# PengfeiRen96/DIR

Measured on AMD Instinct MI355X. Metric: images/sec at 256x256 bs=64, 3 stage outputs (DIR.forward eval), higher is better.
Workload: dtype f16

## Files before the change

### dir_amd/csrc/bneck.hip

```cpp
#include "conv_common.h"

#ifndef DIR_BNECK_RES16
#define DIR_BNECK_RES16 1
#endif

namespace dir {
namespace {

using convk::bf16_t;
using convk::f16s_t;
using convk::Half;
using convk::f32x16;
typedef __attribute__((ext_vector_type(4))) float f32x4;

constexpr int TH = 8, TW = 16, NPX = TH * TW;
constexpr int PH = TH + 2, PWD = TW + 2, NPP = PH * PWD;
constexpr int PPITCH = 144;
constexpr int W2PITCH = 1168;
constexpr int TPITCH = 528;
constexpr int NTHR = 512;
constexpr int NPRE = (NPP * 8 + NTHR - 1) / NTHR;

struct ChainArgs {
    const bf16_t* y1; const bf16_t* res; bf16_t* out; bf16_t* y1n;
    const bf16_t* w2; const float* sc2; const float* sh2;
    const bf16_t* w3; const float* sc3; const float* sh3;
    const bf16_t* w1n; const float* sc1n; const float* sh1n;
    const bf16_t* x2; const bf16_t* wd;
    int B, H, W, tiles_x, tiles_y, ntiles;
    int decim;
};

template <typename H> __device__ __forceinline__ void unpack4(uint2 v, float (&f)[4]) {
    convk::unpack2<H>(v.x, f[0], f[1]);
    convk::unpack2<H>(v.y, f[2], f[3]);
}

template <bool HAS_RES, int N2, bool HAS_DUAL, typename H = bf16_t>
__global__ __launch_bounds__(NTHR, 1) void bneck_chain_kernel(ChainArgs a) {
    convk::half_kernel_init<H>();
    constexpr bool HAS_NEXT = N2 > 0;
    __shared__ __attribute__((aligned(16))) char s_w2[64 * W2PITCH];
    __shared__ __attribute__((aligned(16))) char s_patch[NPP * PPITCH];
    __shared__ __attribute__((aligned(16))) char s_y2[NPX * PPITCH];
    __shared__ __attribute__((aligned(16))) char s_t[64 * TPITCH];
    __shared__ __attribute__((aligned(16))) float s_ss[896];
    const int tid = threadIdx.x, lane = tid & 63, wave = __builtin_amdgcn_readfirstlane(tid >> 6);
    const int l32 = lane & 31, h = lane >> 5;
    const int l16 = lane & 15, g = lane >> 4;

    for (int c = tid; c < 64 * 72; c += NTHR) {
        const int row = c / 72, col = c - row * 72;
        *reinterpret_cast<uint4*>(s_w2 + row * W2PITCH + col * 16) = *reinterpret_cast<const uint4*>(a.w2 + row * 576 + col * 8);
    }
    if (tid < 64) { s_ss[tid] = a.sc2[tid]; s_ss[64 + tid] = a.sh2[tid]; }
    if (tid < 256) { s_ss[128 + tid] = a.sc3[tid]; s_ss[384 + tid] = a.sh3[tid]; }
    if (HAS_NEXT && tid < N2) { s_ss[640 + tid] = a.sc1n[tid]; s_ss[768 + tid] = a.sh1n[tid]; }
    convk::u32x4 w3f[4];
#pragma unroll
    for (int s = 0; s < 4; ++s) w3f[s] = *reinterpret_cast<const convk::u32x4*>(a.w3 + (32 * wave + l32) * 64 + 16 * s + 8 * h);
    convk::u32x4 wdf[HAS_DUAL ? 4 : 1];
    if constexpr (HAS_DUAL) {
#pragma unroll
        for (int s = 0; s < 4; ++s) wdf[s] = *reinterpret_cast<const convk::u32x4*>(a.wd + (32 * wave + l32) * 64 + 16 * s + 8 * h);
    }
    constexpr int NPT = N2 == 128 ? 4 : 2;
    const int ct = N2 == 128 ? wave : (wave >> 1), pt0 = N2 == 128 ? 0 : 2 * (wave & 1);
    convk::u32x4 w1f[HAS_NEXT ? 8 : 1];
    if constexpr (HAS_NEXT) {
#pragma unroll
        for (int s = 0; s < 8; ++s) w1f[s] = *reinterpret_cast<const convk::u32x4*>(a.w1n + (16 * ct + l16) * 256 + 32 * s + 8 * g);
    }

    const int nblk = gridDim.x;
    int t0, tstep, tend;
    if ((nblk & 7) == 0 && a.ntiles % 8 == 0) {
        const int per = a.ntiles >> 3;
        t0 = (blockIdx.x & 7) * per + (blockIdx.x >> 3); tstep = nblk >> 3; tend = ((blockIdx.x & 7) + 1) * per;
    } else { t0 = blockIdx.x; tstep = nblk; tend = a.ntiles; }

    uint4 pre[NPRE];
    unsigned okmask = 0;
    auto origin = [&](int t, int& b, int& y0, int& x0) {
        const int tx = t % a.tiles_x, r = t / a.tiles_x;
        b = r / a.tiles_y; y0 = (r - b * a.tiles_y) * TH; x0 = tx * TW;
    };
    auto fetch = [&](int t) {
        int b, y0, x0;
        origin(t, b, y0, x0);
        okmask = 0;
#pragma unroll
        for (int i = 0; i < NPRE; ++i) {
            const int e = tid + NTHR * i, pp = e >> 3, cc = e & 7;
            const int pr = pp / PWD, pc = pp - pr * PWD;
            const int iy = y0 - 1 + pr, ix = x0 - 1 + pc;
            if (e < NPP * 8 && iy >= 0 && iy < a.H && ix >= 0 && ix < a.W) okmask |= 1u << i;
            const int iyc = min(max(iy, 0), a.H - 1), ixc = min(max(ix, 0), a.W - 1);
            pre[i] = *reinterpret_cast<const uint4*>(a.y1 + (((long long)b * a.H + iyc) * a.W + ixc) * 64 + cc * 8);
        }
    };
    auto stage = [&]() {
#pragma unroll
        for (int i = 0; i < NPRE; ++i) {
            const int e = tid + NTHR * i, pp = e >> 3, cc = e & 7;
            if (e < NPP * 8)
                *reinterpret_cast<uint4*>(s_patch + pp * PPITCH + cc * 16) = (okmask >> i) & 1u ? pre[i] : make_uint4(0u, 0u, 0u, 0u);
        }
    };

    int t = t0;
    if (t < tend) fetch(t);
#pragma unroll
    for (int s = 0; s < 4; ++s) asm volatile("" ::"v"(w3f[s]));
    if constexpr (HAS_DUAL) {
#pragma unroll
        for (int s = 0; s < 4; ++s) asm volatile("" ::"v"(wdf[s]));
    }
    if constexpr (HAS_NEXT) {
#pragma unroll
        for (int s = 0; s < 8; ++s) asm volatile("" ::"v"(w1f[s]));
    }
    if (t < tend) stage();
    __syncthreads();

    const int mt = wave >> 1, nt = wave & 1;
    const int prow = 2 * mt + (l32 >> 4), pcol = l32 & 15;
    const char* pa_b = s_patch + (prow * PWD + pcol) * PPITCH + 16 * h;
    const char* pa_w = s_w2 + (32 * nt + l32) * W2PITCH + 16 * h;

#if DIR_BNECK_RES16
    uint4 xr[2][2][2];
#else
    uint2 xr[2][2][4];
#endif
    auto out_ptr = [&](int mg, int i, int rb, int ry0, int rx0) {
        const int c = tid + NTHR * i, P = 64 * mg + (c >> 5);
        return a.out + (((long long)rb * a.H + ry0 + (P >> 4)) * a.W + rx0 + (P & 15)) * 256 + (c & 31) * 8;
    };

    auto tile = [&](int t) {
        int b, y0, x0;
        origin(t, b, y0, x0);
        const bool more = t + tstep < tend;
        fetch(more ? t + tstep : t);
        if constexpr (HAS_RES) {
#pragma unroll
            for (int mg = 0; mg < 2; ++mg)
#pragma unroll
                for (int j = 0; j < 2; ++j) {
                    const int P = 64 * mg + 32 * j + l32;
#if DIR_BNECK_RES16
                    const bf16_t* rp = a.res + (((long long)b * a.H + y0 + (P >> 4)) * a.W + x0 + (P & 15)) * 256 + 32 * wave + 8 * h;
#pragma unroll
                    for (int jj = 0; jj < 2; ++jj) xr[mg][j][jj] = *reinterpret_cast<const uint4*>(rp + 16 * jj);
#else
                    const bf16_t* rp = a.res + (((long long)b * a.H + y0 + (P >> 4)) * a.W + x0 + (P & 15)) * 256 + 32 * wave + 4 * h;
#pragma unroll
                    for (int q = 0; q < 4; ++q) xr[mg][j][q] = *reinterpret_cast<const uint2*>(rp + 8 * q);
#endif
                }
        }

        uint4 xq0 = make_uint4(0u, 0u, 0u, 0u), xq1 = xq0;
        if constexpr (HAS_DUAL) {
            const int P0 = tid >> 3, P1 = (tid + NTHR) >> 3;
            xq0 = *reinterpret_cast<const uint4*>(a.x2 + (((long long)b * a.H + y0 + (P0 >> 4)) * a.W + x0 + (P0 & 15)) * 64 + (tid & 7) * 8);
            xq1 = *reinterpret_cast<const uint4*>(a.x2 + (((long long)b * a.H + y0 + (P1 >> 4)) * a.W + x0 + (P1 & 15)) * 64 + (tid & 7) * 8);
        }

        {
            f32x16 acc;
#pragma unroll
            for (int r = 0; r < 16; ++r) acc[r] = 0.f;
            uint4 wv[3], pv[3];
            auto ldfrag = [&](int i, int slot) {
                const int tap = i >> 2, s = i & 3, ky = tap / 3, kx = tap - 3 * ky;
                wv[slot] = *reinterpret_cast<const uint4*>(pa_w + tap * 128 + 32 * s);
                pv[slot] = *reinterpret_cast<const uint4*>(pa_b + (ky * PWD + kx) * PPITCH + 32 * s);
            };
            ldfrag(0, 0);
            ldfrag(1, 1);
#pragma unroll
            for (int i = 0; i < 36; ++i) {
                if (i + 2 < 36) ldfrag(i + 2, (i + 2) % 3);
                __builtin_amdgcn_sched_barrier(0);
                acc = Half<H>::mfma32(wv[i % 3], pv[i % 3], acc);
                __builtin_amdgcn_sched_barrier(0);
            }
#pragma unroll
            for (int q = 0; q < 4; ++q) {
                const int c0 = 32 * nt + 8 * q + 4 * h;
                const float4 sc = *reinterpret_cast<const float4*>(s_ss + c0);
                const float4 sh = *reinterpret_cast<const float4*>(s_ss + 64 + c0);
                uint2 o;
                o.x = Half<H>::pack2_relu(fmaf(acc[4 * q], sc.x, sh.x), fmaf(acc[4 * q + 1], sc.y, sh.y));
                o.y = Half<H>::pack2_relu(fmaf(acc[4 * q + 2], sc.z, sh.z), fmaf(acc[4 * q + 3], sc.w, sh.w));
                *reinterpret_cast<uint2*>(s_y2 + (32 * mt + l32) * PPITCH + c0 * 2) = o;
            }
        }
        __syncthreads();
        if constexpr (HAS_DUAL) {
            *reinterpret_cast<uint4*>(s_patch + (tid >> 3) * PPITCH + (tid & 7) * 16) = xq0;
            *reinterpret_cast<uint4*>(s_patch + ((tid + NTHR) >> 3) * PPITCH + (tid & 7) * 16) = xq1;
            __syncthreads();
        }

#pragma unroll
        for (int mg = 0; mg < 2; ++mg) {
            f32x16 accb[2];
            uint4 pvb[2][4];
#pragma unroll
            for (int j = 0; j < 2; ++j)
#pragma unroll
                for (int s = 0; s < 4; ++s)
                    pvb[j][s] = *reinterpret_cast<const uint4*>(s_y2 + (64 * mg + 32 * j + l32) * PPITCH + 32 * s + 16 * h);
#pragma unroll
            for (int j = 0; j < 2; ++j)
#pragma unroll
                for (int r = 0; r < 16; ++r) accb[j][r] = 0.f;
#pragma unroll
            for (int s = 0; s < 4; ++s)
#pragma unroll
                for (int j = 0; j < 2; ++j) accb[j] = Half<H>::mfma32(w3f[s], pvb[j][s], accb[j]);
            if constexpr (HAS_DUAL) {
#pragma unroll
                for (int j = 0; j < 2; ++j)
#pragma unroll
                    for (int s = 0; s < 4; ++s)
                        pvb[j][s] = *reinterpret_cast<const uint4*>(s_patch + (64 * mg + 32 * j + l32) * PPITCH + 32 * s + 16 * h);
#pragma unroll
                for (int s = 0; s < 4; ++s)
#pragma unroll
                    for (int j = 0; j < 2; ++j) accb[j] = Half<H>::mfma32(wdf[s], pvb[j][s], accb[j]);
            }
#pragma unroll
            for (int j = 0; j < 2; ++j) {
#pragma unroll
                for (int q = 0; q < 4; ++q) {
                    const int c0 = 32 * wave + 8 * q + 4 * h;
                    char* tp = s_t + (32 * j + l32) * TPITCH + c0 * 2;
                    const float4 sc = *reinterpret_cast<const float4*>(s_ss + 128 + c0);
                    const float4 sh = *reinterpret_cast<const float4*>(s_ss + 384 + c0);
                    float v[4] = {fmaf(accb[j][4 * q], sc.x, sh.x), fmaf(accb[j][4 * q + 1], sc.y, sh.y),
                                  fmaf(accb[j][4 * q + 2], sc.z, sh.z), fmaf(accb[j][4 * q + 3], sc.w, sh.w)};
                    if constexpr (HAS_RES) {
                        float rv[4];
#if DIR_BNECK_RES16
                        const uint4 c = xr[mg][j][q >> 1];
                        const auto sx = __builtin_amdgcn_permlane32_swap(c.x, c.z, false, false);
                        const auto sy = __builtin_amdgcn_permlane32_swap(c.y, c.w, false, false);
                        unpack4<H>(make_uint2(sx[q & 1], sy[q & 1]), rv);
#else
                        unpack4<H>(xr[mg][j][q], rv);
#endif
#pragma unroll
                        for (int e = 0; e < 4; ++e) v[e] += rv[e];
                    }
                    uint2 o;
                    o.x = Half<H>::pack2_relu(v[0], v[1]);
                    o.y = Half<H>::pack2_relu(v[2], v[3]);
                    *reinterpret_cast<uint2*>(tp) = o;
                }
            }
            __syncthreads();
            if (!a.decim) {
#pragma unroll
                for (int i = 0; i < 4; ++i) {
                    const int c = tid + NTHR * i;
                    *reinterpret_cast<uint4*>(out_ptr(mg, i, b, y0, x0)) = *reinterpret_cast<const uint4*>(s_t + (c >> 5) * TPITCH + (c & 31) * 16);
                }
            } else {
#pragma unroll
                for (int i = 0; i < 4; ++i) {
                    const int c = tid + NTHR * i, P = 64 * mg + (c >> 5), py = P >> 4, px = P & 15;
                    if (((py | px) & 1) == 0)
                        *reinterpret_cast<uint4*>(a.out + (((long long)b * (a.H >> 1) + ((y0 + py) >> 1)) * (a.W >> 1) + ((x0 + px) >> 1)) * 256 + (c & 31) * 8) =
                            *reinterpret_cast<const uint4*>(s_t + (c >> 5) * TPITCH + (c & 31) * 16);
                }
            }
            if constexpr (HAS_NEXT) {
                f32x4 accc[NPT];
#pragma unroll
                for (int u = 0; u < NPT; ++u) accc[u] = f32x4{0.f, 0.f, 0.f, 0.f};
#pragma unroll
                for (int s = 0; s < 8; ++s)
#pragma unroll
                    for (int u = 0; u < NPT; ++u) {
                        const uint4 pv = *reinterpret_cast<const uint4*>(s_t + (16 * (pt0 + u) + l16) * TPITCH + 64 * s + 16 * g);
                        accc[u] = Half<H>::mfma16(w1f[s], pv, accc[u]);
                    }
                const int c0 = 16 * ct + 4 * g;
                const float4 sc = *reinterpret_cast<const float4*>(s_ss + 640 + c0);
                const float4 sh = *reinterpret_cast<const float4*>(s_ss + 768 + c0);
#pragma unroll
                for (int u = 0; u < NPT; ++u) {
                    const int P = 64 * mg + 16 * (pt0 + u) + l16;
                    uint2 o;
                    o.x = Half<H>::pack2_relu(fmaf(accc[u][0], sc.x, sh.x), fmaf(accc[u][1], sc.y, sh.y));
                    o.y = Half<H>::pack2_relu(fmaf(accc[u][2], sc.z, sh.z), fmaf(accc[u][3], sc.w, sh.w));
                    *reinterpret_cast<uint2*>(a.y1n + (((long long)b * a.H + y0 + (P >> 4)) * a.W + x0 + (P & 15)) * N2 + c0) = o;
                }
            }
            if (mg == 0) __syncthreads();
        }
        stage();
        __syncthreads();
    };
    for (; t < tend; t += tstep) tile(t);
}

}
}

extern "C" int dir_bottleneck_chain_forward(const dir_bneck_chain_params* p, const void* y1, const void* residual, const void* x2, void* out,
                                            void* y1_next, int B, int H, int W, void* stream) {
    using namespace dir;
    DIR_REQUIRE(p && y1 && out && B > 0, "dir_bottleneck_chain_forward: bad args");
    DIR_REQUIRE(p->w2 && p->scale2 && p->shift2 && p->w3 && p->scale3 && p->shift3, "dir_bottleneck_chain_forward: missing conv2 / conv3 parameters");
    DIR_REQUIRE(H > 0 && W > 0 && H % TH == 0 && W % TW == 0, "dir_bottleneck_chain_forward: H must be a multiple of 8 and W of 16");
    const bool next = y1_next != nullptr;
    const bool dual = x2 != nullptr;
    DIR_REQUIRE(!dual || (p->wd && !residual), "dir_bottleneck_chain_forward: a second source needs wd and excludes the identity residual");
    DIR_REQUIRE(!next || (p->w1n && p->scale1n && p->shift1n), "dir_bottleneck_chain_forward: y1_next needs the next conv1 parameters");
    ChainArgs a;
    a.y1 = (const convk::bf16_t*)y1; a.res = (const convk::bf16_t*)residual; a.out = (convk::bf16_t*)out; a.y1n = (convk::bf16_t*)y1_next;
    a.w2 = (const convk::bf16_t*)p->w2; a.sc2 = p->scale2; a.sh2 = p->shift2;
    a.w3 = (const convk::bf16_t*)p->w3; a.sc3 = p->scale3; a.sh3 = p->shift3;
    a.w1n = (const convk::bf16_t*)p->w1n; a.sc1n = p->scale1n; a.sh1n = p->shift1n;
    a.x2 = (const convk::bf16_t*)x2; a.wd = (const convk::bf16_t*)p->wd;
    a.B = B; a.H = H; a.W = W; a.tiles_x = W / TW; a.tiles_y = H / TH; a.decim = p->out_decimate ? 1 : 0;
    const long long nt = (long long)B * a.tiles_x * a.tiles_y;
    DIR_REQUIRE(nt < (1ll << 31) && (long long)B * H * W * 256 < (1ll << 40), "dir_bottleneck_chain_forward: too large");
    a.ntiles = (int)nt;
    static int num_cu = 0;
    if (!num_cu) {
        int dev = 0; hipDeviceProp_t pr;
        num_cu = (hipGetDevice(&dev) == hipSuccess && hipGetDeviceProperties(&pr, dev) == hipSuccess) ? pr.multiProcessorCount : 256;
    }
    const int grid = (int)(nt < num_cu ? nt : num_cu);
    hipStream_t s = (hipStream_t)stream;
    const bool res = residual != nullptr;
    const int n2 = next ? p->n_next : 0;
    DIR_REQUIRE(n2 == 0 || n2 == 64 || n2 == 128, "dir_bottleneck_chain_forward: n_next must be 64 or 128");
    DIR_REQUIRE(p->dtype == 0 || p->dtype == DIR_DT_BF16 || p->dtype == DIR_DT_F16, "dir_bottleneck_chain_forward: dtype must be bf16 (or 0) or f16");
    const bool f16 = p->dtype == DIR_DT_F16;
#define DIR_CHAIN(RES_, N2_, DUAL_) do { if (f16) DIR_LAUNCH((bneck_chain_kernel<RES_, N2_, DUAL_, f16s_t>), dim3(grid), dim3(NTHR), 0, s, a); \
                                         else DIR_LAUNCH((bneck_chain_kernel<RES_, N2_, DUAL_, bf16_t>), dim3(grid), dim3(NTHR), 0, s, a); } while (0)
    if (dual) { if (n2 == 128) DIR_CHAIN(false, 128, true); else if (n2) DIR_CHAIN(false, 64, true); else DIR_CHAIN(false, 0, true); }
    else if (res) { if (n2 == 128) DIR_CHAIN(true, 128, false); else if (n2) DIR_CHAIN(true, 64, false); else DIR_CHAIN(true, 0, false); }
    else { if (n2 == 128) DIR_CHAIN(false, 128, false); else if (n2) DIR_CHAIN(false, 64, false); else DIR_CHAIN(false, 0, false); }
#undef DIR_CHAIN
    return check_launch("dir_bottleneck_chain_forward");
}
```

Measured before the change: 28380.

## Batch bottleneck weight preload, template decimation, and hoist residual lane swaps

Loads the conv2 weights and scale/shift vectors into registers before the first patch fetch, so all global loads go out together before they are written to shared memory. Turns output decimation into a template parameter and rewrites the decimated store so every thread writes one vector without a branch. Computes the residual permlane swaps once per row group instead of once per output quad. Adds an optional, disabled-by-default path that issues the next tile's residual and x2 loads early; this costs more registers and adds template instantiations.

```diff
diff --git a/dir_amd/csrc/bneck.hip b/dir_amd/csrc/bneck.hip
--- a/dir_amd/csrc/bneck.hip
+++ b/dir_amd/csrc/bneck.hip
@@ -1,5 +1,11 @@
 #include "conv_common.h"
 
+#ifndef DIR_BNECK_BATCH
+#define DIR_BNECK_BATCH 1
+#endif
+#ifndef DIR_BNECK_LEAD
+#define DIR_BNECK_LEAD 0
+#endif
 #ifndef DIR_BNECK_RES16
 #define DIR_BNECK_RES16 1
 #endif
@@ -28,7 +34,6 @@
     const bf16_t* w1n; const float* sc1n; const float* sh1n;
     const bf16_t* x2; const bf16_t* wd;
     int B, H, W, tiles_x, tiles_y, ntiles;
-    int decim;
 };
 
 template <typename H> __device__ __forceinline__ void unpack4(uint2 v, float (&f)[4]) {
@@ -36,7 +41,7 @@
     convk::unpack2<H>(v.y, f[2], f[3]);
 }
 
-template <bool HAS_RES, int N2, bool HAS_DUAL, typename H = bf16_t>
+template <bool HAS_RES, int N2, bool HAS_DUAL, bool DECIM, typename H = bf16_t>
 __global__ __launch_bounds__(NTHR, 1) void bneck_chain_kernel(ChainArgs a) {
     convk::half_kernel_init<H>();
     constexpr bool HAS_NEXT = N2 > 0;
@@ -49,6 +54,19 @@
     const int l32 = lane & 31, h = lane >> 5;
     const int l16 = lane & 15, g = lane >> 4;
 
+    static_assert(64 * 72 == 9 * NTHR, "w2: nine chunks per thread");
+#if DIR_BNECK_BATCH
+    uint4 w2r[9];
+#pragma unroll
+    for (int i = 0; i < 9; ++i) {
+        const int c = tid + NTHR * i, row = c / 72, col = c - row * 72;
+        w2r[i] = *reinterpret_cast<const uint4*>(a.w2 + row * 576 + col * 8);
+    }
+    const int t64 = tid & 63, t256 = tid & 255, tn2 = HAS_NEXT ? tid & (N2 - 1) : 0;
+    const float v_sc2 = a.sc2[t64], v_sh2 = a.sh2[t64], v_sc3 = a.sc3[t256], v_sh3 = a.sh3[t256];
+    float v_sc1n = 0.f, v_sh1n = 0.f;
+    if constexpr (HAS_NEXT) { v_sc1n = a.sc1n[tn2]; v_sh1n = a.sh1n[tn2]; }
+#else
     for (int c = tid; c < 64 * 72; c += NTHR) {
         const int row = c / 72, col = c - row * 72;
         *reinterpret_cast<uint4*>(s_w2 + row * W2PITCH + col * 16) = *reinterpret_cast<const uint4*>(a.w2 + row * 576 + col * 8);
@@ -56,6 +74,7 @@
     if (tid < 64) { s_ss[tid] = a.sc2[tid]; s_ss[64 + tid] = a.sh2[tid]; }
     if (tid < 256) { s_ss[128 + tid] = a.sc3[tid]; s_ss[384 + tid] = a.sh3[tid]; }
     if (HAS_NEXT && tid < N2) { s_ss[640 + tid] = a.sc1n[tid]; s_ss[768 + tid] = a.sh1n[tid]; }
+#endif
     convk::u32x4 w3f[4];
 #pragma unroll
     for (int s = 0; s < 4; ++s) w3f[s] = *reinterpret_cast<const convk::u32x4*>(a.w3 + (32 * wave + l32) * 64 + 16 * s + 8 * h);
@@ -85,7 +104,7 @@
         const int tx = t % a.tiles_x, r = t / a.tiles_x;
         b = r / a.tiles_y; y0 = (r - b * a.tiles_y) * TH; x0 = tx * TW;
     };
-    auto fetch = [&](int t) {
+    auto fetch = [&](int t, bool live) {
         int b, y0, x0;
         origin(t, b, y0, x0);
         okmask = 0;
@@ -96,7 +115,8 @@
             const int iy = y0 - 1 + pr, ix = x0 - 1 + pc;
             if (e < NPP * 8 && iy >= 0 && iy < a.H && ix >= 0 && ix < a.W) okmask |= 1u << i;
             const int iyc = min(max(iy, 0), a.H - 1), ixc = min(max(ix, 0), a.W - 1);
-            pre[i] = *reinterpret_cast<const uint4*>(a.y1 + (((long long)b * a.H + iyc) * a.W + ixc) * 64 + cc * 8);
+            const long long px = live ? ((long long)b * a.H + iyc) * a.W + ixc : 0;
+            pre[i] = *reinterpret_cast<const uint4*>(a.y1 + px * 64 + cc * 8);
         }
     };
     auto stage = [&]() {
@@ -109,7 +129,18 @@
     };
 
     int t = t0;
-    if (t < tend) fetch(t);
+    if (t >= tend) return;
+    fetch(t, true);
+#if DIR_BNECK_BATCH
+#pragma unroll
+    for (int i = 0; i < 9; ++i) {
+        const int c = tid + NTHR * i, row = c / 72, col = c - row * 72;
+        *reinterpret_cast<uint4*>(s_w2 + row * W2PITCH + col * 16) = w2r[i];
+    }
+    if (tid < 64) { s_ss[tid] = v_sc2; s_ss[64 + tid] = v_sh2; }
+    if (tid < 256) { s_ss[128 + tid] = v_sc3; s_ss[384 + tid] = v_sh3; }
+    if (HAS_NEXT && tid < N2) { s_ss[640 + tid] = v_sc1n; s_ss[768 + tid] = v_sh1n; }
+#endif
 #pragma unroll
     for (int s = 0; s < 4; ++s) asm volatile("" ::"v"(w3f[s]));
     if constexpr (HAS_DUAL) {
@@ -120,7 +151,7 @@
 #pragma unroll
         for (int s = 0; s < 8; ++s) asm volatile("" ::"v"(w1f[s]));
     }
-    if (t < tend) stage();
+    stage();
     __syncthreads();
 
     const int mt = wave >> 1, nt = wave & 1;
@@ -129,7 +160,7 @@
     const char* pa_w = s_w2 + (32 * nt + l32) * W2PITCH + 16 * h;
 
 #if DIR_BNECK_RES16
-    uint4 xr[2][2][2];
+    convk::u32x4 xr[2][2][2];
 #else
     uint2 xr[2][2][4];
 #endif
@@ -138,35 +169,50 @@
         return a.out + (((long long)rb * a.H + ry0 + (P >> 4)) * a.W + rx0 + (P & 15)) * 256 + (c & 31) * 8;
     };
 
-    auto tile = [&](int t) {
+    auto req_res = [&](int mg, int rb, int ry0, int rx0, bool live) {
+#pragma unroll
+        for (int j = 0; j < 2; ++j) {
+            const int P = 64 * mg + 32 * j + l32;
+            const long long px = live ? ((long long)rb * a.H + ry0 + (P >> 4)) * a.W + rx0 + (P & 15) : 0;
+#if DIR_BNECK_RES16
+            const bf16_t* rp = a.res + px * 256 + 32 * wave + 8 * h;
+#pragma unroll
+            for (int jj = 0; jj < 2; ++jj) xr[mg][j][jj] = *reinterpret_cast<const convk::u32x4*>(rp + 16 * jj);
+#else
+            const bf16_t* rp = a.res + px * 256 + 32 * wave + 4 * h;
+#pragma unroll
+            for (int q = 0; q < 4; ++q) xr[mg][j][q] = *reinterpret_cast<const uint2*>(rp + 8 * q);
+#endif
+        }
+    };
+    uint4 xq0 = make_uint4(0u, 0u, 0u, 0u), xq1 = xq0;
+    auto req_x2 = [&](int rb, int ry0, int rx0, bool live) {
+        const int P0 = tid >> 3, P1 = (tid + NTHR) >> 3;
+        const long long px0 = live ? ((long long)rb * a.H + ry0 + (P0 >> 4)) * a.W + rx0 + (P0 & 15) : 0;
+        const long long px1 = live ? ((long long)rb * a.H + ry0 + (P1 >> 4)) * a.W + rx0 + (P1 & 15) : 0;
+        xq0 = *reinterpret_cast<const uint4*>(a.x2 + px0 * 64 + (tid & 7) * 8);
+        xq1 = *reinterpret_cast<const uint4*>(a.x2 + px1 * 64 + (tid & 7) * 8);
+    };
+#if DIR_BNECK_LEAD
+    {
+        int b, y0, x0;
+        origin(t, b, y0, x0);
+        if constexpr (HAS_RES) { req_res(0, b, y0, x0, true); req_res(1, b, y0, x0, true); }
+        if constexpr (HAS_DUAL) req_x2(b, y0, x0, true);
+    }
+#endif
+
+    auto tile = [&](int t) __attribute__((always_inline)) {
         int b, y0, x0;
         origin(t, b, y0, x0);
         const bool more = t + tstep < tend;
-        fetch(more ? t + tstep : t);
-        if constexpr (HAS_RES) {
-#pragma unroll
-            for (int mg = 0; mg < 2; ++mg)
-#pragma unroll
-                for (int j = 0; j < 2; ++j) {
-                    const int P = 64 * mg + 32 * j + l32;
-#if DIR_BNECK_RES16
-                    const bf16_t* rp = a.res + (((long long)b * a.H + y0 + (P >> 4)) * a.W + x0 + (P & 15)) * 256 + 32 * wave + 8 * h;
-#pragma unroll
-                    for (int jj = 0; jj < 2; ++jj) xr[mg][j][jj] = *reinterpret_cast<const uint4*>(rp + 16 * jj);
-#else
-                    const bf16_t* rp = a.res + (((long long)b * a.H + y0 + (P >> 4)) * a.W + x0 + (P & 15)) * 256 + 32 * wave + 4 * h;
-#pragma unroll
-                    for (int q = 0; q < 4; ++q) xr[mg][j][q] = *reinterpret_cast<const uint2*>(rp + 8 * q);
-#endif
-                }
-        }
-
-        uint4 xq0 = make_uint4(0u, 0u, 0u, 0u), xq1 = xq0;
-        if constexpr (HAS_DUAL) {
-            const int P0 = tid >> 3, P1 = (tid + NTHR) >> 3;
-            xq0 = *reinterpret_cast<const uint4*>(a.x2 + (((long long)b * a.H + y0 + (P0 >> 4)) * a.W + x0 + (P0 & 15)) * 64 + (tid & 7) * 8);
-            xq1 = *reinterpret_cast<const uint4*>(a.x2 + (((long long)b * a.H + y0 + (P1 >> 4)) * a.W + x0 + (P1 & 15)) * 64 + (tid & 7) * 8);
-        }
+        int bn, yn0, xn0;
+        origin(more ? t + tstep : t, bn, yn0, xn0);
+        fetch(more ? t + tstep : t, more);
+#if !DIR_BNECK_LEAD
+        if constexpr (HAS_RES) { req_res(0, b, y0, x0, true); req_res(1, b, y0, x0, true); }
+        if constexpr (HAS_DUAL) req_x2(b, y0, x0, true);
+#endif
 
         {
             f32x16 acc;
@@ -202,6 +248,11 @@
         if constexpr (HAS_DUAL) {
             *reinterpret_cast<uint4*>(s_patch + (tid >> 3) * PPITCH + (tid & 7) * 16) = xq0;
             *reinterpret_cast<uint4*>(s_patch + ((tid + NTHR) >> 3) * PPITCH + (tid & 7) * 16) = xq1;
+#if DIR_BNECK_LEAD
+            __builtin_amdgcn_sched_barrier(0);
+            req_x2(bn, yn0, xn0, more);
+            __builtin_amdgcn_sched_barrier(0);
+#endif
             __syncthreads();
         }
 
@@ -235,6 +286,22 @@
             }
 #pragma unroll
             for (int j = 0; j < 2; ++j) {
+#if DIR_BNECK_RES16
+                uint2 rq[4];
+                if constexpr (HAS_RES) {
+#pragma unroll
+                    for (int jj = 0; jj < 2; ++jj) {
+                        convk::u32x4 c = xr[mg][j][jj];
+#if DIR_BNECK_LEAD
+                        asm volatile("" : "+v"(c));
+#endif
+                        const auto sx = __builtin_amdgcn_permlane32_swap(c[0], c[2], false, false);
+                        const auto sy = __builtin_amdgcn_permlane32_swap(c[1], c[3], false, false);
+                        rq[2 * jj] = make_uint2(sx[0], sy[0]);
+                        rq[2 * jj + 1] = make_uint2(sx[1], sy[1]);
+                    }
+                }
+#endif
 #pragma unroll
                 for (int q = 0; q < 4; ++q) {
                     const int c0 = 32 * wave + 8 * q + 4 * h;
@@ -246,10 +313,7 @@
                     if constexpr (HAS_RES) {
                         float rv[4];
 #if DIR_BNECK_RES16
-                        const uint4 c = xr[mg][j][q >> 1];
-                        const auto sx = __builtin_amdgcn_permlane32_swap(c.x, c.z, false, false);
-                        const auto sy = __builtin_amdgcn_permlane32_swap(c.y, c.w, false, false);
-                        unpack4<H>(make_uint2(sx[q & 1], sy[q & 1]), rv);
+                        unpack4<H>(rq[q], rv);
 #else
                         unpack4<H>(xr[mg][j][q], rv);
 #endif
@@ -262,21 +326,24 @@
                     *reinterpret_cast<uint2*>(tp) = o;
                 }
             }
+#if DIR_BNECK_LEAD
+            if constexpr (HAS_RES) {
+                __builtin_amdgcn_sched_barrier(0);
+                req_res(mg, bn, yn0, xn0, more);
+                __builtin_amdgcn_sched_barrier(0);
+            }
+#endif
             __syncthreads();
-            if (!a.decim) {
+            if constexpr (!DECIM) {
 #pragma unroll
                 for (int i = 0; i < 4; ++i) {
                     const int c = tid + NTHR * i;
                     *reinterpret_cast<uint4*>(out_ptr(mg, i, b, y0, x0)) = *reinterpret_cast<const uint4*>(s_t + (c >> 5) * TPITCH + (c & 31) * 16);
                 }
             } else {
-#pragma unroll
-                for (int i = 0; i < 4; ++i) {
-                    const int c = tid + NTHR * i, P = 64 * mg + (c >> 5), py = P >> 4, px = P & 15;
-                    if (((py | px) & 1) == 0)
-                        *reinterpret_cast<uint4*>(a.out + (((long long)b * (a.H >> 1) + ((y0 + py) >> 1)) * (a.W >> 1) + ((x0 + px) >> 1)) * 256 + (c & 31) * 8) =
-                            *reinterpret_cast<const uint4*>(s_t + (c >> 5) * TPITCH + (c & 31) * 16);
-                }
+                const int k = tid >> 5, py = 4 * mg + 2 * (k >> 3), px = 2 * (k & 7);
+                *reinterpret_cast<uint4*>(a.out + (((long long)b * (a.H >> 1) + ((y0 + py) >> 1)) * (a.W >> 1) + ((x0 + px) >> 1)) * 256 + (tid & 31) * 8) =
+                    *reinterpret_cast<const uint4*>(s_t + (32 * (k >> 3) + px) * TPITCH + (tid & 31) * 16);
             }
             if constexpr (HAS_NEXT) {
                 f32x4 accc[NPT];
@@ -306,6 +373,10 @@
         stage();
         __syncthreads();
     };
+#if DIR_BNECK_LEAD
+    tile(t);
+    t += tstep;
+#endif
     for (; t < tend; t += tstep) tile(t);
 }
 
@@ -328,7 +399,7 @@
     a.w3 = (const convk::bf16_t*)p->w3; a.sc3 = p->scale3; a.sh3 = p->shift3;
     a.w1n = (const convk::bf16_t*)p->w1n; a.sc1n = p->scale1n; a.sh1n = p->shift1n;
     a.x2 = (const convk::bf16_t*)x2; a.wd = (const convk::bf16_t*)p->wd;
-    a.B = B; a.H = H; a.W = W; a.tiles_x = W / TW; a.tiles_y = H / TH; a.decim = p->out_decimate ? 1 : 0;
+    a.B = B; a.H = H; a.W = W; a.tiles_x = W / TW; a.tiles_y = H / TH;
     const long long nt = (long long)B * a.tiles_x * a.tiles_y;
     DIR_REQUIRE(nt < (1ll << 31) && (long long)B * H * W * 256 < (1ll << 40), "dir_bottleneck_chain_forward: too large");
     a.ntiles = (int)nt;
@@ -344,11 +415,14 @@
     DIR_REQUIRE(n2 == 0 || n2 == 64 || n2 == 128, "dir_bottleneck_chain_forward: n_next must be 64 or 128");
     DIR_REQUIRE(p->dtype == 0 || p->dtype == DIR_DT_BF16 || p->dtype == DIR_DT_F16, "dir_bottleneck_chain_forward: dtype must be bf16 (or 0) or f16");
     const bool f16 = p->dtype == DIR_DT_F16;
-#define DIR_CHAIN(RES_, N2_, DUAL_) do { if (f16) DIR_LAUNCH((bneck_chain_kernel<RES_, N2_, DUAL_, f16s_t>), dim3(grid), dim3(NTHR), 0, s, a); \
-                                         else DIR_LAUNCH((bneck_chain_kernel<RES_, N2_, DUAL_, bf16_t>), dim3(grid), dim3(NTHR), 0, s, a); } while (0)
+    const bool decim = p->out_decimate != 0;
+#define DIR_CHAIN_D(RES_, N2_, DUAL_, DEC_) do { if (f16) DIR_LAUNCH((bneck_chain_kernel<RES_, N2_, DUAL_, DEC_, f16s_t>), dim3(grid), dim3(NTHR), 0, s, a); \
+                                                 else DIR_LAUNCH((bneck_chain_kernel<RES_, N2_, DUAL_, DEC_, bf16_t>), dim3(grid), dim3(NTHR), 0, s, a); } while (0)
+#define DIR_CHAIN(RES_, N2_, DUAL_) do { if (decim) DIR_CHAIN_D(RES_, N2_, DUAL_, true); else DIR_CHAIN_D(RES_, N2_, DUAL_, false); } while (0)
     if (dual) { if (n2 == 128) DIR_CHAIN(false, 128, true); else if (n2) DIR_CHAIN(false, 64, true); else DIR_CHAIN(false, 0, true); }
     else if (res) { if (n2 == 128) DIR_CHAIN(true, 128, false); else if (n2) DIR_CHAIN(true, 64, false); else DIR_CHAIN(true, 0, false); }
     else { if (n2 == 128) DIR_CHAIN(false, 128, false); else if (n2) DIR_CHAIN(false, 64, false); else DIR_CHAIN(false, 0, false); }
 #undef DIR_CHAIN
+#undef DIR_CHAIN_D
     return check_launch("dir_bottleneck_chain_forward");
 }
```

After: 28390 (median of 5 runs). No clear change (+0.0%).
